# SUSTech-SLAM-XYZZY/SurfelMapping

Measured on AMD Instinct MI355X. Metric: frames/sec per GPU, 1242x375 KITTI-shaped RGB-D+semantic, full associate+fuse+merge, higher is better.
Workload: dtype f32; 1 GPU; BASELINE configs[1]: KITTI 1242x375 synthetic street sequence, 0.8 m/frame, depth noise 15.0 mm, metricise+conflict+cull+splat+associate+fuse+append per frame; frames=5..6245, multi_gpu=single stream, surfels_start=157613, surfels_end=5487352

## Files before the change

surfelmapping_amd/csrc/sm_device.h:

```cpp
#pragma once

#include <hip/hip_runtime.h>
#include <stdint.h>

namespace sm {

constexpr uint64_t KEY_EMPTY = 0x7FFFFFFFFFFFFFFFull;
constexpr int TILE = 1024;
constexpr int TILE_WORDS = TILE / 64;
constexpr int PIX_BLOCK = 256;
constexpr int SUB_STRIDE = 32;
constexpr int SUB_SET = 64 * SUB_STRIDE;

struct SurfelSet {
    float4 *pos_conf;
    float4 *norm_rad;
    uint32_t *color;
    float *init_time;
    float *time;
};

struct Model {
    SurfelSet s[2];
};

struct DevState {
    uint32_t count;
    uint32_t offset;
    uint32_t cur;
    uint32_t cull_n;
    uint32_t cull_src, cull_dst;
    uint32_t n_kill;
    uint32_t conflict_count;
    uint32_t data_count, unstable_count, fused_count;
    uint32_t visible_count;
    uint32_t append_n;
    int32_t error;
    uint32_t frames_logged;
    uint32_t n_static;
    uint32_t n_conf_skipped;
    uint32_t n_splat_skipped;
    uint32_t garbage;
    uint32_t garbage_prev;
    uint32_t do_compact;
    uint32_t cap_binds;
    uint32_t first_moving;
    uint32_t compact_ticket;
    uint32_t stat_frames;
    uint32_t first_live;
    uint32_t fl_dirty2[2];
    uint32_t slow_frames;
    uint32_t slow_done[2];
    uint32_t pend;
    uint32_t pend_tick;
    uint32_t holes_last;
};

struct FrameLog { uint32_t tick, n_before, n_after_cull, n_kill, conflict_count, visible_count, fused_count, unstable_count, n_static, n_conf_skipped, n_splat_skipped, n_slots; };
constexpr uint32_t FRAME_LOG_LEN = 1024;

struct FrameParams {
    float pose[16];
    float t_inv[16];
    float fx, fy, cx, cy;
    float inv_fx, inv_fy;
    float cols, rows;
    int W, H, P;
    float min_depth, max_depth;
    float conflict_thresh;
    float fuse_thresh;
    float stereo_border;
    int is_clean;
    int time;
    int time_delta;
    float depth_cutoff;
    uint32_t conflict_cap;
    int splat_follows;
    int log_frame;
    uint32_t max_vertices;
    int init_mode;
    float inv_fx_fb, inv_fy_fb;
    int use_bounds;
    uint32_t compact_now;
    int maintenance;
    int compact_tickets;
    int no_exempt;
    int shard_slots;
    int par;
};

__device__ __forceinline__ float min_glsl(float a, float b) { return (b < a) ? b : a; }

__device__ __forceinline__ int tex_idx(float t, int n)
{
    float f = floorf(t * (float)n);
    if (!(f >= 0.0f)) return 0;
    if (f > (float)(n - 1)) return n - 1;
    return (int)f;
}

__device__ __forceinline__ float3 xform3(const float *m, float x, float y, float z)
{
    float3 r;
    r.x = ((m[0] * x + m[4] * y) + m[8] * z) + m[12];
    r.y = ((m[1] * x + m[5] * y) + m[9] * z) + m[13];
    r.z = ((m[2] * x + m[6] * y) + m[10] * z) + m[14];
    return r;
}

__device__ __forceinline__ float3 rot3(const float *m, float x, float y, float z)
{
    float3 r;
    r.x = (m[0] * x + m[4] * y) + m[8] * z;
    r.y = (m[1] * x + m[5] * y) + m[9] * z;
    r.z = (m[2] * x + m[6] * y) + m[10] * z;
    return r;
}

__device__ __forceinline__ float dot3(float3 a, float3 b) { return (a.x * b.x + a.y * b.y) + a.z * b.z; }

__device__ __forceinline__ float3 cross3(float3 a, float3 b)
{
    float3 r;
    r.x = a.y * b.z - a.z * b.y;
    r.y = a.z * b.x - a.x * b.z;
    r.z = a.x * b.y - a.y * b.x;
    return r;
}

__device__ __forceinline__ float3 normalize3(float3 v)
{
    float l = sqrtf(dot3(v, v));
    float3 r;
    r.x = v.x / l; r.y = v.y / l; r.z = v.z / l;
    return r;
}

__device__ __forceinline__ float acos_spec(float x)
{
    const float pS0 = 1.6666586697e-01f, pS1 = -4.2743422091e-02f, pS2 = -8.6563630030e-03f;
    const float qS1 = -7.0662963390e-01f;
    const float PIO2 = 1.57079637050628662109375f, PI = 3.1415927410125732421875f;
    float ax = fabsf(x);
    if (ax <= 0.5f) {
        float z = x * x;
        float r = (z * (pS0 + z * (pS1 + z * pS2))) / (1.0f + z * qS1);
        return PIO2 - (x + x * r);
    } else if (x > 0.0f) {
        float z = (1.0f - x) * 0.5f;
        float s = sqrtf(z);
        float r = (z * (pS0 + z * (pS1 + z * pS2))) / (1.0f + z * qS1);
        return 2.0f * (s + s * r);
    } else {
        float z = (1.0f + x) * 0.5f;
        float s = sqrtf(z);
        float r = (z * (pS0 + z * (pS1 + z * pS2))) / (1.0f + z * qS1);
        return PI - 2.0f * (s + s * r);
    }
}

__device__ __forceinline__ uint32_t round_u8(float v)
{
    float r = roundf(v);
    if (!(r >= 0.0f)) return 0u;
    if (r > 4294967040.0f) return 4294967040u;
    return (uint32_t)r;
}

__device__ __forceinline__ uint32_t encode_color(float r, float g, float b, uint32_t sem)
{
    uint32_t srgb = sem;
    srgb = (srgb << 8) + round_u8(r * 255.0f);
    srgb = (srgb << 8) + round_u8(g * 255.0f);
    srgb = (srgb << 8) + round_u8(b * 255.0f);
    return srgb;
}

__device__ __forceinline__ float get_radius(float depth, float norm_z, float inv_fx, float inv_fy)
{
    float meanFocal = ((1.0f / fabsf(inv_fx)) + (1.0f / fabsf(inv_fy))) / 2.0f;
    const float sqrt2 = 1.41421356237f;
    float radius = (depth / meanFocal) * sqrt2;
    float radius_n = radius / fabsf(norm_z);
    return min_glsl(2.0f * radius, radius_n);
}

__device__ __forceinline__ uint32_t block_scan_1024(uint32_t v, uint32_t *total, uint32_t *lds)
{
    const int lane = threadIdx.x & 63, wave = threadIdx.x >> 6;
    uint32_t inc = v;
#pragma unroll
    for (int o = 1; o < 64; o <<= 1) {
        uint32_t t = __shfl_up(inc, o);
        if (lane >= o) inc += t;
    }
    if (lane == 63) lds[wave] = inc;
    __syncthreads();
    if (wave == 0) {
        uint32_t w = lane < 16 ? lds[lane] : 0u;
        uint32_t wi = w;
#pragma unroll
        for (int o = 1; o < 16; o <<= 1) {
            uint32_t t = __shfl_up(wi, o);
            if (lane >= o) wi += t;
        }
        if (lane < 16) lds[lane] = wi - w;
        if (lane == 15) lds[16] = wi;
    }
    __syncthreads();
    uint32_t excl = inc - v + lds[wave];
    *total = lds[16];
    __syncthreads();
    return excl;
}

__device__ __forceinline__ uint32_t f2ord(float f)
{
    const uint32_t b = __float_as_uint(f);
    return (b & 0x80000000u) ? ~b : (b | 0x80000000u);
}
__device__ __forceinline__ float ord2f(uint32_t o)
{
    return __uint_as_float((o & 0x80000000u) ? (o & 0x7FFFFFFFu) : ~o);
}

__device__ __forceinline__ uint32_t lane_bcast(uint32_t v, int l)
{
    return (uint32_t)__builtin_amdgcn_readlane((int)v, __builtin_amdgcn_readfirstlane(l));
}

template <int CTRL, int ROW_MASK>
__device__ __forceinline__ uint32_t dpp_take(uint32_t v)
{
    return (uint32_t)__builtin_amdgcn_update_dpp(0, (int)v, CTRL, ROW_MASK, 0xF, true);
}
__device__ __forceinline__ uint32_t wave_max_u32(uint32_t v)
{
    v = max(v, dpp_take<0x111, 0xF>(v));
    v = max(v, dpp_take<0x112, 0xF>(v));
    v = max(v, dpp_take<0x114, 0xF>(v));
    v = max(v, dpp_take<0x118, 0xF>(v));
    v = max(v, dpp_take<0x142, 0xA>(v));
    v = max(v, dpp_take<0x143, 0xC>(v));
    return (uint32_t)__builtin_amdgcn_readlane((int)v, 63);
}
__device__ __forceinline__ uint32_t wave_sum_u32(uint32_t v)
{
    v += dpp_take<0x111, 0xF>(v);
    v += dpp_take<0x112, 0xF>(v);
    v += dpp_take<0x114, 0xF>(v);
    v += dpp_take<0x118, 0xF>(v);
    v += dpp_take<0x142, 0xA>(v);
    v += dpp_take<0x143, 0xC>(v);
    return (uint32_t)__builtin_amdgcn_readlane((int)v, 63);
}

__device__ __forceinline__ bool slow_frame(const DevState *__restrict__ st, const uint32_t *__restrict__ conf_sub, uint32_t cap, int par, int lane)
{
    const uint32_t ctotal = wave_sum_u32(conf_sub[lane * SUB_STRIDE]);
    return ctotal > cap || st->fl_dirty2[par] != 0u;
}

__device__ __forceinline__ void wait_slow_frame(DevState *__restrict__ st, int par, uint32_t need)
{
    uint32_t spins = 0;
    while (__hip_atomic_load(&st->slow_done[par], __ATOMIC_ACQUIRE, __HIP_MEMORY_SCOPE_AGENT) < need) {
        __builtin_amdgcn_s_sleep(8);
        if (++spins > (1u << 22)) { st->error = -6; break; }
    }
}


__device__ __forceinline__ void bounds_expand_wave(uint32_t *__restrict__ tb, bool active, uint32_t tile, float x, float y,
                                                   float z, float t, bool bad)
{
    uint64_t todo = __ballot(active);
    const int lane = threadIdx.x & 63;
    while (todo) {
        const int leader = __ffsll((long long)todo) - 1;
        const uint32_t tcur = (uint32_t)__shfl((int)tile, leader);
        const bool mine = active && tile == tcur;
        const uint64_t grp = __ballot(mine);
        uint32_t w0 = mine ? ~f2ord(x) : 0u, w1 = mine ? ~f2ord(y) : 0u, w2 = mine ? ~f2ord(z) : 0u;
        uint32_t w4 = mine ? f2ord(x) : 0u, w5 = mine ? f2ord(y) : 0u, w6 = mine ? f2ord(z) : 0u, w7 = mine ? f2ord(t) : 0u;
        const uint32_t nb = (uint32_t)__popcll(__ballot(mine && (bad || x != x || y != y || z != z)));
        w0 = wave_max_u32(w0); w1 = wave_max_u32(w1); w2 = wave_max_u32(w2); w4 = wave_max_u32(w4);
        w5 = wave_max_u32(w5); w6 = wave_max_u32(w6); w7 = wave_max_u32(w7);
        if (lane < 8 && lane != 3) {
            const uint32_t val = lane == 0 ? w0 : lane == 1 ? w1 : lane == 2 ? w2 : lane == 4 ? w4 : lane == 5 ? w5 : lane == 6 ? w6 : w7;
            atomicMax(&tb[(size_t)tcur * 8 + lane], val);
        }
        if (nb && lane == 3) atomicAdd(&tb[(size_t)tcur * 8 + 3], nb);
        todo &= ~grp;
    }
}

__device__ __forceinline__ bool box_outside_view(const uint32_t *__restrict__ b, const float *t_inv, float fx, float fy, float cx,
                                                 float cy, float zlo, float zhi, float ulo, float uhi, float vlo, float vhi)
{
    if (b[3] != 0u) return false;
    if (b[0] == 0u && b[4] == 0u) return true;
    const float lx = ord2f(~b[0]), ly = ord2f(~b[1]), lz = ord2f(~b[2]), hx = ord2f(b[4]), hy = ord2f(b[5]), hz = ord2f(b[6]);
    float zmin = 3.0e38f, zmax = -3.0e38f;
    bool all_right = true, all_left = true, all_below = true, all_above = true, finite = true;
#pragma unroll
    for (int c = 0; c < 8; ++c) {
        const float3 p = xform3(t_inv, (c & 1) ? hx : lx, (c & 2) ? hy : ly, (c & 4) ? hz : lz);
        finite = finite && (p.x - p.x == 0.0f) && (p.y - p.y == 0.0f) && (p.z - p.z == 0.0f);
        zmin = fminf(zmin, p.z); zmax = fmaxf(zmax, p.z);
        all_right = all_right && (fx * p.x + (cx - uhi - 2.0f) * p.z > 0.0f);
        all_left = all_left && (fx * p.x + (cx - ulo + 2.0f) * p.z < 0.0f);
        all_below = all_below && (fy * p.y + (cy - vhi - 2.0f) * p.z > 0.0f);
        all_above = all_above && (fy * p.y + (cy - vlo + 2.0f) * p.z < 0.0f);
    }
    if (!finite) return false;
    if (zmax < zlo - 0.01f || zmin > zhi + 0.01f) return true;
    if (zmin > 1.0e-3f && (all_right || all_left || all_below || all_above)) return true;
    return false;
}

__device__ __forceinline__ uint64_t first_n_bits(uint64_t m, uint32_t n)
{
    if (n >= (uint32_t)__popcll(m)) return m;
    uint64_t rest = m;
    for (uint32_t i = 0; i < n; ++i) rest &= rest - 1;
    return m ^ rest;
}

}
```

surfelmapping_amd/csrc/sm_k_cull.h:

```cpp
#pragma once

#ifndef SM_CONFLICT_WAVES
#define SM_CONFLICT_WAVES 5
#endif
__global__ __launch_bounds__(256) __attribute__((amdgpu_waves_per_eu(SM_CONFLICT_WAVES, 8))) void k_conflict(Model M, const DevState *__restrict__ st, FrameParams fp,
                                                  const uint2 *__restrict__ dcT ,
                                                  uint64_t *__restrict__ cm, uint64_t *__restrict__ dm,
                                                  uint64_t *__restrict__ zm, uint32_t *__restrict__ tile_cnt,
                                                  const uint32_t *__restrict__ tb, uint8_t *__restrict__ tile_flags,
                                                  uint32_t *__restrict__ blk_part ,
                                                  const uint64_t *__restrict__ alive,
                                                  uint32_t *__restrict__ conf_sub )
{
    __shared__ uint32_t s_red[4][3];
    __shared__ uint64_t s_m[3][TILE_WORDS];
    __shared__ uint8_t s_flags[64];
    const uint32_t N = st->count;
    const bool has_dead = st->garbage != 0u;
    const uint32_t exempt = fp.no_exempt ? 0xFFFFFFFFu : st->first_live;
    const float4 *__restrict__ pc = M.s[st->cur].pos_conf;
    const uint32_t ntiles = (N + TILE - 1) / TILE;
    const int lane = threadIdx.x & 63, wave = threadIdx.x >> 6;
    uint32_t skipped = 0;
    uint32_t acc = 0;
    uint64_t skipmask = 0;
    uint32_t iter = 0;
    for (uint32_t tile = blockIdx.x; tile < ntiles; tile += gridDim.x, ++iter) {
        uint32_t nconf = 0, nkill = 0, nzero = 0;
        if ((iter & 63u) == 0u) {
            __syncthreads();
            tile_flags_batch(tile, gridDim.x, ntiles, fp, tb, s_flags);
            __syncthreads();
            const uint64_t tl = (uint64_t)tile + (uint64_t)lane * gridDim.x;
            const uint32_t f = s_flags[lane];
            if (wave == 0 && tl < ntiles) tile_flags[tl] = (uint8_t)f;
            skipmask = __ballot((f & 1u) != 0u);
        }
        if ((skipmask >> (iter & 63u)) & 1ull) {
            if (threadIdx.x < 3) tile_cnt[tile * 3 + threadIdx.x] = 0u;
            if (threadIdx.x >= 64 && threadIdx.x < 64 + 3 * TILE_WORDS) {
                const int m = (threadIdx.x - 64) / TILE_WORDS, w = (threadIdx.x - 64) % TILE_WORDS;
                const uint32_t word = tile * TILE_WORDS + w;
                if ((uint64_t)word * 64u < N) { uint64_t *dst = m == 0 ? cm : (m == 1 ? dm : zm); dst[word] = 0ull; }
            }
            skipped += min((uint32_t)TILE, N - tile * TILE);
            continue;
        }
        float4 v[4];
        bool valid[4];
#pragma unroll
        for (int r = 0; r < 4; ++r) {
            const uint32_t k = (tile * TILE_WORDS + r * 4 + wave) * 64u + lane;
            valid[r] = k < N;
            v[r] = pc[min(k, N - 1u)];
        }
        if (has_dead) {
#pragma unroll
            for (int r = 0; r < 4; ++r) valid[r] = valid[r] && ((alive[tile * TILE_WORDS + r * 4 + wave] >> lane) & 1ull);
        }
        float zc[4], lam[4], dep[4];
        uint32_t cls[4], qq[4];
        bool inview[4];
#pragma unroll
        for (int r = 0; r < 4; ++r) {
            inview[r] = false; zc[r] = 0.f; lam[r] = 0.f; qq[r] = 0u;
            if (valid[r]) {
                const float3 ph = xform3(fp.t_inv, v[r].x, v[r].y, v[r].z);
                if (!(ph.z <= fp.min_depth || ph.z >= fp.max_depth)) {
                    const float xl = ph.x / ph.z;
                    const float yl = ph.y / ph.z;
                    const float u = fp.fx * xl + fp.cx;
                    const float vv = fp.fy * yl + fp.cy;
                    if (!(u < fp.stereo_border || u > fp.cols || vv < 0.0f || vv > fp.rows)) {
                        const int ti = tex_idx(u / fp.cols, fp.W), tj = tex_idx(vv / fp.rows, fp.H);
                        qq[r] = (uint32_t)(ti * fp.H + tj);
                        lam[r] = sqrtf((xl * xl + yl * yl) + 1.0f);
                        zc[r] = ph.z;
                        inview[r] = true;
                    }
                }
            }
        }
#pragma unroll
        for (int r = 0; r < 4; ++r) {
            const uint2 g = dcT[qq[r]];
            dep[r] = __uint_as_float(g.x);
            cls[r] = g.y >> 24;
        }
#pragma unroll
        for (int r = 0; r < 4; ++r) {
            const uint32_t word = tile * TILE_WORDS + r * 4 + wave;
            const uint32_t k = word * 64u + lane;
            bool conflict = false;
            if (inview[r]) {
                float depth = dep[r];
                if (cls[r] == 10u) depth = fp.max_depth + 1.0f;
                if (fp.is_clean == 0 && depth == 0.0f) depth = fp.max_depth + 20.0f;
                conflict = (depth * lam[r] - zc[r] * lam[r] > fp.conflict_thresh * zc[r]) && (k != exempt);
            }
            const bool dies = valid[r] && !(v[r].w - 1.0f > 0.0f);
            const bool dead = valid[r] && !(v[r].w > 0.0f);
            const uint64_t cw = __ballot(conflict), dw = __ballot(dies), zw = __ballot(dead);
            if (lane == 0) { s_m[0][r * 4 + wave] = cw; s_m[1][r * 4 + wave] = dw; s_m[2][r * 4 + wave] = zw; }
            nconf += __popcll(cw);
            nkill += __popcll(zw | (cw & dw));
            nzero += __popcll(zw);
        }
        if (lane == 0) { s_red[wave][0] = nconf; s_red[wave][1] = nkill; s_red[wave][2] = nzero; }
        __syncthreads();
        if (threadIdx.x < 3) {
            const uint32_t tsum = s_red[0][threadIdx.x] + s_red[1][threadIdx.x] + s_red[2][threadIdx.x] + s_red[3][threadIdx.x];
            tile_cnt[tile * 3 + threadIdx.x] = tsum;
            acc += tsum;
        }
        if (threadIdx.x >= 64 && threadIdx.x < 64 + 3 * TILE_WORDS) {
            const int m = (threadIdx.x - 64) / TILE_WORDS, w = (threadIdx.x - 64) % TILE_WORDS;
            const uint32_t word = tile * TILE_WORDS + w;
            if ((uint64_t)word * 64u < N) {
                uint64_t *dst = m == 0 ? cm : (m == 1 ? dm : zm);
                dst[word] = s_m[m][w];
            }
        }
        __syncthreads();
    }
    if (threadIdx.x < 2) blk_part[blockIdx.x * 4 + 1 + threadIdx.x] = acc;
    if (threadIdx.x == 0) {
        blk_part[blockIdx.x * 4] = skipped;
        if (acc) atomicAdd(&conf_sub[(blockIdx.x & 63u) * SUB_STRIDE], acc);
    }
}

constexpr int GROUP = 1024;

__global__ __launch_bounds__(1024) void k_scan_cull(const DevState *__restrict__ st,
                                                    const uint32_t *__restrict__ tile_cnt,
                                                    uint32_t *__restrict__ tile_allow,
                                                    uint32_t *__restrict__ tile_keep_prefix,
                                                    uint32_t *__restrict__ group_tot ,
                                                    const uint32_t *__restrict__ tile_dead)
{
    __shared__ uint32_t s_scan[17];
    __shared__ uint32_t s_first;
    const uint32_t N = st->count;
    const uint32_t ntiles = (N + TILE - 1) / TILE;
    const uint32_t t = blockIdx.x * GROUP + threadIdx.x;
    if (threadIdx.x == 0) s_first = 0xFFFFFFFFu;
    uint32_t nconf = 0, keep = 0;
    bool kills = false;
    if (t < ntiles) {
        nconf = tile_cnt[t * 3];
        const uint32_t nkill = tile_cnt[t * 3 + 1];
        keep = min((uint32_t)TILE, N - t * TILE) - tile_dead[t] - nkill;
        kills = nkill != 0 || tile_dead[t] != 0;
        tile_allow[t] = nconf;
    }
    uint32_t ctot, ktot;
    block_scan_1024(nconf, &ctot, s_scan);
    const uint32_t kpre = block_scan_1024(keep, &ktot, s_scan);
    if (kills) atomicMin(&s_first, t);
    if (t < ntiles) tile_keep_prefix[t] = kpre;
    __syncthreads();
    if (threadIdx.x == 0) {
        group_tot[blockIdx.x * 4 + 0] = ctot;
        group_tot[blockIdx.x * 4 + 1] = ktot;
        group_tot[blockIdx.x * 4 + 2] = s_first;
    }
}

__device__ __forceinline__ uint64_t keep_word(uint32_t t, int w, uint32_t N, const uint64_t *__restrict__ cm,
                                              const uint64_t *__restrict__ dm, const uint64_t *__restrict__ zm,
                                              const uint64_t *__restrict__ alive, uint32_t allow, uint32_t nconf)
{
    const uint32_t word = t * TILE_WORDS + (uint32_t)w;
    const uint64_t base = (uint64_t)word * 64u;
    if (base >= N) return 0ull;
    const uint64_t rem = (uint64_t)N - base;
    const uint64_t valid = (rem >= 64 ? ~0ull : ((1ull << rem) - 1ull)) & alive[word];
    uint64_t ce = cm[word];
    if (allow != nconf) {
        uint32_t before = 0;
        for (int x = 0; x < w; ++x) before += (uint32_t)__popcll(cm[t * TILE_WORDS + x]);
        ce = before >= allow ? 0ull : first_n_bits(ce, allow - before);
    }
    return ~(zm[word] | (ce & dm[word])) & valid;
}

__global__ __launch_bounds__(1024) void k_cull_finalize(DevState *__restrict__ st, FrameParams fp,
                                                        const uint64_t *__restrict__ cm,
                                                        const uint64_t *__restrict__ dm,
                                                        const uint64_t *__restrict__ zm,
                                                        const uint32_t *__restrict__ tile_cnt,
                                                        uint32_t *__restrict__ tile_allow,
                                                        uint32_t *__restrict__ tile_keep_prefix,
                                                        const uint32_t *__restrict__ group_tot,
                                                        uint32_t *__restrict__ group_keep_base,
                                                        const uint32_t *__restrict__ conf_part, uint32_t n_conf_part,
                                                        const uint64_t *__restrict__ alive,
                                                        const uint32_t *__restrict__ tile_dead,
                                                        unsigned long long *__restrict__ host_stat)
{
    __shared__ uint32_t s_scan[17];
    __shared__ uint32_t s_first, s_ft, s_fl, s_keep_first;
    const uint32_t N = st->count;
    const uint32_t g0 = st->garbage;
    const uint32_t old_first = st->first_live, old_offset = st->offset;
    const uint32_t holes = st->holes_last;
    const uint32_t ntiles = (N + TILE - 1) / TILE;
    const uint32_t ngroups = (ntiles + GROUP - 1) / GROUP;
    const uint32_t cap = fp.conflict_cap;
    const bool have_scan = fp.compact_now != 0u || fp.maintenance != 0;
    if (threadIdx.x == 0) { s_first = 0xFFFFFFFFu; s_ft = 0xFFFFFFFFu; s_fl = 0xFFFFFFFFu; }
    if (threadIdx.x == 1023) {
        uint32_t survive = 0;
        if (old_first < N) {
            const uint32_t w = old_first / 64u, bit = old_first % 64u;
            survive = (((zm[w] | (cm[w] & dm[w])) >> bit) & 1ull) ? 0u : 1u;
        }
        s_keep_first = survive;
    }
    uint32_t cskip = 0, cconf = 0, ckill = 0, cskip_tot, cconf_tot, ckill_tot;
    for (uint32_t b = threadIdx.x; b < n_conf_part; b += 1024u) {
        cskip += conf_part[b * 4]; cconf += conf_part[b * 4 + 1]; ckill += conf_part[b * 4 + 2];
    }
    __syncthreads();
    block_scan_1024(cskip, &cskip_tot, s_scan);
    block_scan_1024(cconf, &cconf_tot, s_scan);
    block_scan_1024(ckill, &ckill_tot, s_scan);
    uint32_t ctotal = cconf_tot, ktotal = (N - g0) - ckill_tot, gkpre = 0;
    uint32_t nstatic = N;
    if (have_scan) {
        uint32_t gc = 0, gk = 0;
        if (threadIdx.x < ngroups) {
            gc = group_tot[threadIdx.x * 4 + 0];
            gk = group_tot[threadIdx.x * 4 + 1];
            atomicMin(&s_first, group_tot[threadIdx.x * 4 + 2]);
        }
        block_scan_1024(gc, &ctotal, s_scan);
        gkpre = block_scan_1024(gk, &ktotal, s_scan);
        nstatic = (s_first == 0xFFFFFFFFu) ? N : min(N, s_first * (uint32_t)TILE);
    }
    const bool cap_binds = ctotal > cap;
    if (!cap_binds) {
        if (have_scan && threadIdx.x < ngroups) group_keep_base[threadIdx.x] = gkpre;
    } else {
        if (threadIdx.x < ngroups) group_keep_base[threadIdx.x] = 0;
        const uint32_t per = (ntiles + 1023u) / 1024u;
        const uint32_t t0 = min(threadIdx.x * per, ntiles), t1 = min(t0 + per, ntiles);
        uint32_t csum = 0;
        for (uint32_t t = t0; t < t1; ++t) csum += tile_cnt[t * 3];
        uint32_t dummy;
        uint32_t cpre = block_scan_1024(csum, &dummy, s_scan);
        uint32_t ksum = 0;
        for (uint32_t t = t0; t < t1; ++t) {
            const uint32_t nconf = tile_cnt[t * 3];
            uint32_t allow = nconf;
            if (cpre >= cap) allow = 0;
            else if (cap - cpre < nconf) allow = cap - cpre;
            tile_allow[t] = allow;
            uint32_t kills;
            if (allow == nconf) kills = tile_cnt[t * 3 + 1];
            else if (allow == 0) kills = tile_cnt[t * 3 + 2];
            else {
                kills = 0;
                uint32_t rem = allow;
                for (int w = 0; w < TILE_WORDS; ++w) {
                    const uint32_t word = t * TILE_WORDS + w;
                    if ((uint64_t)word * 64u >= N) break;
                    const uint64_t c = cm[word];
                    const uint64_t ce = first_n_bits(c, rem);
                    rem -= (uint32_t)__popcll(ce);
                    kills += (uint32_t)__popcll(zm[word] | (ce & dm[word]));
                }
            }
            tile_keep_prefix[t] = kills;
            ksum += min((uint32_t)TILE, N - t * TILE) - tile_dead[t] - kills;
            cpre += nconf;
        }
        uint32_t kpre = block_scan_1024(ksum, &ktotal, s_scan);
        uint32_t ns = 0;
        for (uint32_t t = t0; t < t1; ++t) {
            const uint32_t kills = tile_keep_prefix[t];
            const uint32_t nv = min((uint32_t)TILE, N - t * TILE) - tile_dead[t];
            if (kpre == t * TILE && kills == 0 && tile_dead[t] == 0u) ns += nv;
            else atomicMin(&s_first, t);
            tile_keep_prefix[t] = kpre;
            kpre += nv - kills;
        }
        block_scan_1024(ns, &nstatic, s_scan);
        __syncthreads();
    }
    const uint32_t kept = ktotal;
    const uint32_t g1 = N - kept;
    const bool compact = have_scan;
    uint32_t first_live = compact ? 0u : N;
    if (!compact && kept != 0u) {
        __syncthreads();
        if (s_keep_first) {
            first_live = old_first;
        } else {
            for (uint32_t base = min(old_first, N - 1u) / TILE; base < ntiles; base += 1024u) {
                const uint32_t t = base + threadIdx.x;
                if (t < ntiles) {
                    uint32_t keep_t;
                    if (cap_binds) keep_t = ((t + 1 < ntiles) ? tile_keep_prefix[t + 1] : kept) - tile_keep_prefix[t];
                    else keep_t = min((uint32_t)TILE, N - t * TILE) - tile_dead[t] - tile_cnt[t * 3 + 1];
                    if (keep_t != 0u) atomicMin(&s_ft, t);
                }
                __syncthreads();
                const uint32_t found = s_ft;
                __syncthreads();
                if (found != 0xFFFFFFFFu) break;
            }
            const uint32_t ft = s_ft;
            if (ft != 0xFFFFFFFFu && threadIdx.x < TILE_WORDS) {
                const uint32_t nconf = tile_cnt[ft * 3];
                const uint64_t k = keep_word(ft, (int)threadIdx.x, N, cm, dm, zm, alive, cap_binds ? tile_allow[ft] : nconf, nconf);
                if (k) atomicMin(&s_fl, (ft * TILE_WORDS + threadIdx.x) * 64u + (uint32_t)(__ffsll((long long)k) - 1));
            }
            __syncthreads();
            first_live = s_fl;
        }
    }
    if (threadIdx.x == 0) {
        if (!fp.maintenance) {
            st->n_conf_skipped = cskip_tot;
            st->n_static = compact ? nstatic : N;
            st->n_kill = (N - g0) - kept;
            st->conflict_count = min(ctotal, cap);
            if (fp.splat_follows) st->visible_count = 0;
        }
        st->cull_n = N;
        st->cull_src = st->cur;
        st->cull_dst = st->cur;
        st->garbage_prev = g0;
        st->cap_binds = cap_binds ? 1u : 0u;
        st->do_compact = compact ? 1u : 0u;
        st->first_moving = (compact && s_first != 0xFFFFFFFFu) ? min(s_first, ntiles) : ntiles;
        st->compact_ticket = 0u;
        st->first_live = first_live;
        st->fl_dirty2[0] = 0u; st->fl_dirty2[1] = 0u;
        st->slow_done[0] = 0u; st->slow_done[1] = 0u;
        st->holes_last = 0u;
        if (compact) {
            st->count = kept;
            st->offset = fp.maintenance ? old_offset - (g0 - holes) : kept;
            st->garbage = 0;
        } else {
            st->count = N;
            st->offset = N;
            st->garbage = g1;
        }
        if (host_stat)
            __hip_atomic_store(host_stat, ((unsigned long long)st->stat_frames << 32) | (unsigned long long)(compact ? kept : N),
                               __ATOMIC_RELAXED, __HIP_MEMORY_SCOPE_SYSTEM);
    }
}

__device__ __forceinline__ void post_compact_fill(const DevState *__restrict__ st, uint64_t *__restrict__ alive,
                                                  uint32_t *__restrict__ tile_dead, uint32_t tid, uint32_t nthreads)
{
    if (st->do_compact == 0u || st->garbage_prev == 0u) return;
    const uint32_t n = st->cull_n;
    const uint32_t nwords = (n + 63u) / 64u, ntiles = (n + TILE - 1) / TILE;
    for (uint32_t w = tid; w < nwords; w += nthreads) alive[w] = ~0ull;
    for (uint32_t t = tid; t < ntiles; t += nthreads) tile_dead[t] = 0u;
}

__global__ void k_post_fill(const DevState *__restrict__ st, uint64_t *__restrict__ alive, uint32_t *__restrict__ tile_dead)
{
    post_compact_fill(st, alive, tile_dead, blockIdx.x * blockDim.x + threadIdx.x, gridDim.x * blockDim.x);
}

__global__ void k_remap_keys(const DevState *__restrict__ st, uint64_t *__restrict__ keyT, int P,
                             const uint64_t *__restrict__ alive, const uint32_t *__restrict__ tile_keep_prefix,
                             const uint32_t *__restrict__ group_keep_base)
{
    const int q = blockIdx.x * blockDim.x + threadIdx.x;
    if (q >= P || st->garbage_prev == 0u) return;
    const uint64_t key = keyT[q];
    if (key == KEY_EMPTY) return;
    const uint32_t id = (uint32_t)(key & 0xFFFFFFFFull);
    if (id >= st->cull_n) return;
    const uint32_t tile = id / TILE, w = (id % TILE) / 64u, bit = id % 64u;
    uint32_t nid = tile_keep_prefix[tile] + group_keep_base[tile / GROUP];
    for (uint32_t x = 0; x < w; ++x) nid += (uint32_t)__popcll(alive[tile * TILE_WORDS + x]);
    nid += (uint32_t)__popcll(alive[tile * TILE_WORDS + w] & ((1ull << bit) - 1ull));
    keyT[q] = (key & 0xFFFFFFFF00000000ull) | (uint64_t)nid;
}

__device__ __forceinline__ bool splat_one(const FrameParams &fp, float x, float y, float z, float t_last,
                                          uint32_t id, uint64_t *__restrict__ keyT)
{
    const float3 ph = xform3(fp.t_inv, x, y, z);
    if (ph.z >= fp.depth_cutoff * 1.5f || ph.z <= 0.0f || (float)fp.time - t_last > (float)fp.time_delta)
        return false;
    const float xn = ((((fp.fx * ph.x) / ph.z) + fp.cx) - (fp.cols * 0.5f)) / (fp.cols * 0.5f);
    const float yn = ((((fp.fy * ph.y) / ph.z) + fp.cy) - (fp.rows * 0.5f)) / (fp.rows * 0.5f);
    const float zn = ph.z / fp.depth_cutoff;
    if (!(xn >= -1.0f && xn <= 1.0f && yn >= -1.0f && yn <= 1.0f && zn >= -1.0f && zn <= 1.0f)) return false;
    const float xw = (fp.cols * 0.5f) * xn + (fp.cols * 0.5f);
    const float yw = (fp.rows * 0.5f) * yn + (fp.rows * 0.5f);
    const float fxw = floorf(xw), fyw = floorf(yw);
    if (!(fxw >= 0.0f && fxw < fp.cols && fyw >= 0.0f && fyw < fp.rows)) return false;
    const int px = (int)fxw, py = (int)fyw;
    const float zw = 0.5f * zn + 0.5f;
    const uint32_t d24 = (uint32_t)floor((double)zw * 16777215.0 + 0.5);
    if (d24 >= 16777215u) return false;
    const uint64_t key = ((uint64_t)d24 << 32) | (uint64_t)id;
    atomicMin((unsigned long long *)&keyT[(size_t)px * fp.H + py], (unsigned long long)key);
    return true;
}

template <bool SPLAT>
__global__ __launch_bounds__(256) void k_compact(Model M, DevState *__restrict__ st, FrameParams fp,
                                                 const uint64_t *__restrict__ cm,
                                                 const uint64_t *__restrict__ dm,
                                                 const uint64_t *__restrict__ zm,
                                                 const uint32_t *__restrict__ tile_cnt,
                                                 const uint32_t *__restrict__ tile_allow,
                                                 const uint32_t *__restrict__ tile_keep_prefix,
                                                 uint64_t *__restrict__ keyT,
                                                 uint32_t *__restrict__ tile_flag, uint32_t epoch,
                                                 const uint32_t *__restrict__ group_keep_base,
                                                 uint32_t *__restrict__ tb, const uint8_t *__restrict__ tile_flags,
                                                 uint2 *__restrict__ blk_part ,
                                                 uint64_t *__restrict__ alive, uint32_t *__restrict__ tile_dead)
{
    __shared__ uint64_t s_keep[TILE_WORDS], s_ceff[TILE_WORDS];
    __shared__ uint32_t s_cpop[TILE_WORDS], s_kpre[TILE_WORDS + 1];
    __shared__ uint32_t s_vis[4];
    const uint32_t N = st->cull_n;
    const SurfelSet set = M.s[st->cull_src];
    const uint32_t ntiles = (N + TILE - 1) / TILE;
    const int lane = threadIdx.x & 63, wave = threadIdx.x >> 6;
    uint32_t vis = 0, skipped = 0, iter = 0;
    uint64_t skipmask = 0;
    uint32_t m_nconf = 0, m_nkill = 0, m_allow = 0, m_base = 0, m_dead = 0;
    const bool had_dead = st->garbage_prev != 0u;
    const bool cap_binds = st->cap_binds != 0u;
    const bool use_tickets = fp.compact_tickets != 0;
    const uint32_t fm = use_tickets ? min(st->first_moving, ntiles) : ntiles;
    constexpr uint32_t TICKET = 1;
    __shared__ uint32_t s_tk;
    bool ticketing = false;
    uint32_t rr_tile = blockIdx.x, tk_tile = 0, tk_left = 0;
    for (;;) {
        uint32_t tile, allow, nconf, nkill_full, base_id, tdead;
        bool skipbit;
        if (!ticketing && rr_tile >= fm) {
            if (!use_tickets) break;
            ticketing = true;
        }
        if (!ticketing) {
            tile = rr_tile;
            if ((iter & 63u) == 0u) {
                const uint64_t tl = (uint64_t)tile + (uint64_t)lane * gridDim.x;
                const bool in = tl < fm;
                const uint32_t tt = in ? (uint32_t)tl : 0u;
                skipmask = __ballot(in && (tile_flags[tt] & 2u));
                m_nconf = tile_cnt[tt * 3]; m_nkill = tile_cnt[tt * 3 + 1];
                m_allow = cap_binds ? tile_allow[tt] : m_nconf;
                m_base = tile_keep_prefix[tt] + group_keep_base[tt / GROUP];
                m_dead = had_dead ? tile_dead[tt] : 0u;
            }
            const int sl = (int)(iter & 63u);
            allow = lane_bcast(m_allow, sl); nconf = lane_bcast(m_nconf, sl);
            nkill_full = lane_bcast(m_nkill, sl); base_id = lane_bcast(m_base, sl);
            tdead = lane_bcast(m_dead, sl);
            skipbit = (skipmask >> (iter & 63u)) & 1ull;
            rr_tile += gridDim.x; ++iter;
        } else {
            if (tk_left == 0u) {
                __syncthreads();
                if (threadIdx.x == 0) s_tk = atomicAdd(&st->compact_ticket, TICKET);
                __syncthreads();
                tk_tile = fm + s_tk; tk_left = TICKET;
            }
            tile = tk_tile;
            if (tile >= ntiles) break;
            ++tk_tile; --tk_left;
            nconf = tile_cnt[tile * 3]; nkill_full = tile_cnt[tile * 3 + 1];
            allow = cap_binds ? tile_allow[tile] : nconf;
            base_id = tile_keep_prefix[tile] + group_keep_base[tile / GROUP];
            tdead = had_dead ? tile_dead[tile] : 0u;
            skipbit = false;
        }
        if (!ticketing && nconf == 0 && nkill_full == 0 && base_id == tile * (uint32_t)TILE && tdead == 0u) {
            if (SPLAT && skipbit) {
                skipped += min((uint32_t)TILE, N - tile * TILE);
                continue;
            }
            if (SPLAT) {
                float4 pv[4];
                float pt[4];
#pragma unroll
                for (int r = 0; r < 4; ++r) {
                    const uint32_t k = (tile * TILE_WORDS + r * 4 + wave) * 64u + lane;
                    const uint32_t kc = min(k, N - 1u);
                    pv[r] = set.pos_conf[kc];
                    pt[r] = set.time[kc];
                }
#pragma unroll
                for (int r = 0; r < 4; ++r) {
                    const uint32_t k = (tile * TILE_WORDS + r * 4 + wave) * 64u + lane;
                    bool drew = false;
                    if (k < N)
                        drew = splat_one(fp, pv[r].x, pv[r].y, pv[r].z, pt[r], k, keyT);
                    vis += (uint32_t)__popcll(__ballot(drew));
                }
            }
            continue;
        }
        const bool moving = ticketing || (base_id != tile * (uint32_t)TILE) || nkill_full != 0u || tdead != 0u;
        float4 v[4], nr[4];
        uint32_t col[4], nid[4];
        float it[4], tl[4];
        bool kept[4];
#pragma unroll
        for (int r = 0; r < 4; ++r) {
            const uint32_t k = (tile * TILE_WORDS + r * 4 + wave) * 64u + lane;
            const uint32_t kc = min(k, N - 1u);
            v[r] = set.pos_conf[kc];
            tl[r] = set.time[kc];
            nr[r] = make_float4(0.f, 0.f, 0.f, 0.f); col[r] = 0; it[r] = 0.f;
            if (moving) { nr[r] = set.norm_rad[kc]; col[r] = set.color[kc]; it[r] = set.init_time[kc]; }
        }
        uint64_t c = 0, d = 0, z = 0, valid = 0;
        if (threadIdx.x < TILE_WORDS) {
            const uint32_t word = tile * TILE_WORDS + threadIdx.x;
            const uint64_t base = (uint64_t)word * 64u;
            if (base < N) {
                c = cm[word]; d = dm[word]; z = zm[word];
                const uint64_t rem = (uint64_t)N - base;
                valid = rem >= 64 ? ~0ull : ((1ull << rem) - 1ull);
                if (had_dead) valid &= alive[word];
            }
            s_cpop[threadIdx.x] = (uint32_t)__popcll(c);
        }
        __syncthreads();
        if (threadIdx.x < TILE_WORDS) {
            uint64_t ce = c;
            if (allow != nconf) {
                uint32_t before = 0;
                for (int w = 0; w < (int)threadIdx.x; ++w) before += s_cpop[w];
                ce = before >= allow ? 0ull : first_n_bits(c, allow - before);
            }
            const uint64_t keep = ~(z | (ce & d)) & valid;
            s_ceff[threadIdx.x] = ce;
            s_keep[threadIdx.x] = keep;
        }
        __syncthreads();
        if (threadIdx.x <= TILE_WORDS) {
            uint32_t before = 0;
            for (int w = 0; w < (int)threadIdx.x; ++w) before += (uint32_t)__popcll(s_keep[w]);
            s_kpre[threadIdx.x] = before;
        }
        __syncthreads();
        const uint32_t kcount = s_kpre[TILE_WORDS];
#pragma unroll
        for (int r = 0; r < 4; ++r) {
            const int w = r * 4 + wave;
            const uint64_t keepw = s_keep[w];
            kept[r] = (keepw >> lane) & 1ull;
            nid[r] = base_id + s_kpre[w] + (uint32_t)__popcll(keepw & ((1ull << lane) - 1ull));
            if (kept[r] && ((s_ceff[w] >> lane) & 1ull)) {
                v[r].w -= 1.0f;
                if (!moving) set.pos_conf[(tile * TILE_WORDS + w) * 64u + lane].w = v[r].w;
            }
        }
        if (moving) {
            if (threadIdx.x < 8) atomicExch(&tb[(size_t)tile * 8 + threadIdx.x], 0u);
            asm volatile("s_waitcnt vmcnt(0)" ::: "memory");
            __syncthreads();
            if (threadIdx.x == 0) {
                __hip_atomic_exchange(&tile_flag[tile], epoch, __ATOMIC_RELAXED, __HIP_MEMORY_SCOPE_AGENT);
                if (kcount && base_id != tile * TILE) {
                    const uint32_t first = base_id / TILE;
                    const uint32_t last = min(tile - 1u, (base_id + kcount - 1u) / TILE);
                    for (uint32_t t = first; t <= last; ++t) {
                        uint32_t spins = 0;
                        while (__hip_atomic_load(&tile_flag[t], __ATOMIC_RELAXED, __HIP_MEMORY_SCOPE_AGENT) != epoch) {
                            __builtin_amdgcn_s_sleep(2);
                            if (++spins > (1u << 24)) { st->error = -6; break; }
                        }
                    }
                }
            }
            __syncthreads();
#pragma unroll
            for (int r = 0; r < 4; ++r) {
                if (kept[r]) {
                    set.pos_conf[nid[r]] = v[r];
                    set.norm_rad[nid[r]] = nr[r];
                    set.color[nid[r]] = col[r];
                    set.init_time[nid[r]] = it[r];
                    set.time[nid[r]] = tl[r];
                }
                bounds_expand_wave(tb, kept[r], nid[r] / (uint32_t)TILE, v[r].x, v[r].y, v[r].z, tl[r], false);
            }
        }
        if (SPLAT) {
#pragma unroll
            for (int r = 0; r < 4; ++r) {
                bool drew = false;
                if (kept[r])
                    drew = splat_one(fp, v[r].x, v[r].y, v[r].z, tl[r], nid[r], keyT);
                vis += (uint32_t)__popcll(__ballot(drew));
            }
        }
        __syncthreads();
    }
    if (SPLAT) {
        if (lane == 0) s_vis[wave] = vis;
        __syncthreads();
        if (threadIdx.x == 0)
            blk_part[blockIdx.x] = make_uint2(s_vis[0] + s_vis[1] + s_vis[2] + s_vis[3], skipped);
    }
}

__global__ __launch_bounds__(256) void k_cull_lazy(Model M, const DevState *__restrict__ st, FrameParams fp,
                                                   const uint64_t *__restrict__ cm, const uint64_t *__restrict__ dm,
                                                   const uint64_t *__restrict__ zm, const uint32_t *__restrict__ tile_cnt,
                                                   const uint32_t *__restrict__ tile_allow,
                                                   uint64_t *__restrict__ alive, uint32_t *__restrict__ tile_dead)
{
    const uint32_t N = st->cull_n;
    const SurfelSet set = M.s[st->cull_src];
    const uint32_t ntiles = (N + TILE - 1) / TILE;
    const int lane = threadIdx.x & 63, wave = threadIdx.x >> 6;
    const bool had_dead = st->garbage_prev != 0u, cap_binds = st->cap_binds != 0u;
    uint32_t iter = 0;
    uint32_t m_nconf = 0, m_nkill = 0, m_dead = 0;
    for (uint32_t tile = blockIdx.x; tile < ntiles; tile += gridDim.x, ++iter) {
        if ((iter & 63u) == 0u) {
            const uint64_t tl = (uint64_t)tile + (uint64_t)lane * gridDim.x;
            const bool in = tl < ntiles;
            const uint32_t tt = in ? (uint32_t)tl : 0u;
            m_nconf = tile_cnt[tt * 3]; m_nkill = tile_cnt[tt * 3 + 1];
            m_dead = had_dead ? tile_dead[tt] : 0u;
        }
        const int sl = (int)(iter & 63u);
        const uint32_t nconf = lane_bcast(m_nconf, sl), nkill = lane_bcast(m_nkill, sl);
        const uint32_t tdead = lane_bcast(m_dead, sl);
        const bool touched = nconf != 0u || nkill != 0u;
        if (!touched) continue;
        float4 pv[4];
#pragma unroll
        for (int r = 0; r < 4; ++r) {
            const uint32_t kc = min((tile * TILE_WORDS + r * 4 + wave) * 64u + lane, N - 1u);
            pv[r] = set.pos_conf[kc];
        }
        const uint32_t allow = (touched && cap_binds) ? tile_allow[tile] : nconf;
        uint32_t killed = 0;
#pragma unroll
        for (int r = 0; r < 4; ++r) {
            const int w = r * 4 + wave;
            const uint32_t word = tile * TILE_WORDS + (uint32_t)w;
            const uint32_t k = word * 64u + lane;
            const uint64_t base = (uint64_t)word * 64u;
            uint64_t range = 0ull;
            if (base < N) { const uint64_t rem = (uint64_t)N - base; range = rem >= 64 ? ~0ull : ((1ull << rem) - 1ull); }
            const uint64_t valid = range & ((tdead != 0u) ? alive[word] : ~0ull);
            uint64_t keep = valid, ce = 0ull;
            if (touched) {
                ce = cm[word];
                if (allow != nconf) {
                    uint32_t before = 0;
                    for (int x = 0; x < w; ++x) before += (uint32_t)__popcll(cm[tile * TILE_WORDS + x]);
                    ce = before >= allow ? 0ull : first_n_bits(ce, allow - before);
                }
                keep = ~(zm[word] | (ce & dm[word])) & valid;
                if (keep != valid && lane == 0) alive[word] = keep | ~range;
                killed += (uint32_t)__popcll(valid ^ keep);
            }
            const bool kp = (keep >> lane) & 1ull;
            if (kp && ((ce >> lane) & 1ull)) set.pos_conf[k].w = pv[r].w - 1.0f;
        }
        if (killed && lane == 0) atomicAdd(&tile_dead[tile], killed);
    }
}
```

Baseline: 25550 frames/s.

## Prefetch alive bitmask words and redirect dead-lane loads to live slots

In the conflict and cull/compact kernels, the per-wave alive bitmask words for the next tile are now loaded one iteration ahead, with the wave index made scalar via readfirstlane so the loads stay uniform. Lanes whose surfel is dead have their gather address redirected to the first live slot in the same word, so dead lanes add no extra cache lines to the surfel attribute loads. The conflict kernel's waves-per-EU hint also goes from 5 to 6. This adds register pressure for the prefetched words and a little address logic per load.

```diff
diff --git a/surfelmapping_amd/csrc/sm_device.h b/surfelmapping_amd/csrc/sm_device.h
--- a/surfelmapping_amd/csrc/sm_device.h
+++ b/surfelmapping_amd/csrc/sm_device.h
@@ -327,4 +327,9 @@
     return m ^ rest;
 }
 
-}
+__device__ __forceinline__ uint32_t live_slot(uint64_t a, int lane, uint32_t k, uint32_t word_base, uint32_t N)
+{
+    return ((a >> lane) & 1ull) ? k : min(word_base + (a ? (uint32_t)__builtin_ctzll(a) : 0u), N - 1u);
+}
+
+}
diff --git a/surfelmapping_amd/csrc/sm_k_cull.h b/surfelmapping_amd/csrc/sm_k_cull.h
--- a/surfelmapping_amd/csrc/sm_k_cull.h
+++ b/surfelmapping_amd/csrc/sm_k_cull.h
@@ -1,7 +1,7 @@
 #pragma once
 
 #ifndef SM_CONFLICT_WAVES
-#define SM_CONFLICT_WAVES 5
+#define SM_CONFLICT_WAVES 6
 #endif
 __global__ __launch_bounds__(256) __attribute__((amdgpu_waves_per_eu(SM_CONFLICT_WAVES, 8))) void k_conflict(Model M, const DevState *__restrict__ st, FrameParams fp,
                                                   const uint2 *__restrict__ dcT ,
@@ -25,8 +25,21 @@
     uint32_t acc = 0;
     uint64_t skipmask = 0;
     uint32_t iter = 0;
+    const uint32_t wv = (uint32_t)__builtin_amdgcn_readfirstlane(wave);
+    uint64_t a_next[4] = {~0ull, ~0ull, ~0ull, ~0ull};
+    if (has_dead && blockIdx.x < ntiles) {
+#pragma unroll
+        for (int r = 0; r < 4; ++r) a_next[r] = alive[blockIdx.x * TILE_WORDS + r * 4 + wv];
+    }
     for (uint32_t tile = blockIdx.x; tile < ntiles; tile += gridDim.x, ++iter) {
         uint32_t nconf = 0, nkill = 0, nzero = 0;
+        uint64_t aw[4];
+#pragma unroll
+        for (int r = 0; r < 4; ++r) aw[r] = a_next[r];
+        if (has_dead && tile + gridDim.x < ntiles) {
+#pragma unroll
+            for (int r = 0; r < 4; ++r) a_next[r] = alive[(tile + gridDim.x) * TILE_WORDS + r * 4 + wv];
+        }
         if ((iter & 63u) == 0u) {
             __syncthreads();
             tile_flags_batch(tile, gridDim.x, ntiles, fp, tb, s_flags);
@@ -50,13 +63,9 @@
         bool valid[4];
 #pragma unroll
         for (int r = 0; r < 4; ++r) {
-            const uint32_t k = (tile * TILE_WORDS + r * 4 + wave) * 64u + lane;
-            valid[r] = k < N;
-            v[r] = pc[min(k, N - 1u)];
-        }
-        if (has_dead) {
-#pragma unroll
-            for (int r = 0; r < 4; ++r) valid[r] = valid[r] && ((alive[tile * TILE_WORDS + r * 4 + wave] >> lane) & 1ull);
+            const uint32_t wbase = (tile * TILE_WORDS + r * 4 + wave) * 64u, k = wbase + lane;
+            valid[r] = k < N && ((aw[r] >> lane) & 1ull);
+            v[r] = pc[live_slot(aw[r], lane, min(k, N - 1u), wbase, N)];
         }
         float zc[4], lam[4], dep[4];
         uint32_t cls[4], qq[4];
@@ -444,9 +453,16 @@
     __shared__ uint32_t s_tk;
     bool ticketing = false;
     uint32_t rr_tile = blockIdx.x, tk_tile = 0, tk_left = 0;
+    const uint32_t wv = (uint32_t)__builtin_amdgcn_readfirstlane(wave);
+    uint64_t a_next[4] = {~0ull, ~0ull, ~0ull, ~0ull};
+    if (had_dead && blockIdx.x < fm) {
+#pragma unroll
+        for (int r = 0; r < 4; ++r) a_next[r] = alive[blockIdx.x * TILE_WORDS + r * 4 + wv];
+    }
     for (;;) {
         uint32_t tile, allow, nconf, nkill_full, base_id, tdead;
         bool skipbit;
+        uint64_t aw[4];
         if (!ticketing && rr_tile >= fm) {
             if (!use_tickets) break;
             ticketing = true;
@@ -469,6 +485,12 @@
             tdead = lane_bcast(m_dead, sl);
             skipbit = (skipmask >> (iter & 63u)) & 1ull;
             rr_tile += gridDim.x; ++iter;
+#pragma unroll
+            for (int r = 0; r < 4; ++r) aw[r] = a_next[r];
+            if (had_dead && rr_tile < fm) {
+#pragma unroll
+                for (int r = 0; r < 4; ++r) a_next[r] = alive[rr_tile * TILE_WORDS + r * 4 + wv];
+            }
         } else {
             if (tk_left == 0u) {
                 __syncthreads();
@@ -484,6 +506,8 @@
             base_id = tile_keep_prefix[tile] + group_keep_base[tile / GROUP];
             tdead = had_dead ? tile_dead[tile] : 0u;
             skipbit = false;
+#pragma unroll
+            for (int r = 0; r < 4; ++r) aw[r] = had_dead ? alive[tile * TILE_WORDS + r * 4 + wv] : ~0ull;
         }
         if (!ticketing && nconf == 0 && nkill_full == 0 && base_id == tile * (uint32_t)TILE && tdead == 0u) {
             if (SPLAT && skipbit) {
@@ -518,8 +542,8 @@
         bool kept[4];
 #pragma unroll
         for (int r = 0; r < 4; ++r) {
-            const uint32_t k = (tile * TILE_WORDS + r * 4 + wave) * 64u + lane;
-            const uint32_t kc = min(k, N - 1u);
+            const uint32_t wbase = (tile * TILE_WORDS + r * 4 + wave) * 64u;
+            const uint32_t kc = live_slot(aw[r], lane, min(wbase + lane, N - 1u), wbase, N);
             v[r] = set.pos_conf[kc];
             tl[r] = set.time[kc];
             nr[r] = make_float4(0.f, 0.f, 0.f, 0.f); col[r] = 0; it[r] = 0.f;
```

Measured after the change: 25340 frames/s (median of 6 runs). About the same (-0.8%).
